# snakers4/mnasnet-pytorch

Measured on AMD Instinct MI355X. Metric: images/sec MNASNet-1.0 224^2 bf16 train step, higher is better.
Workload: dtype bf16; 1 GPU; MNASNet-1.0 (Mnasnet(cut_channels_first=False)+head '512', 1000 classes) fwd+bwd+Adam, bs=256/GPU, 224x224, per-rank BatchNorm; global_batch=256, parallelism=dp1

## Files before the change

### include/mnas.h

```cpp
#ifndef MNAS_H
#define MNAS_H
#include <stdint.h>

#ifdef __cplusplus
extern "C" {
#endif

#define MNAS_OK 0
#define MNAS_EINVAL 10001
#define MNAS_BN_ROWS 8

typedef struct MnasActIn {
    const void*  data;
    const float* scale;
    const float* shift;
} MnasActIn;

typedef struct MnasGradIn {
    const void*  g;
    const void*  y;
    const float* coef;
} MnasGradIn;

int mnas_version(void);
// ... 52 lines not shown

typedef struct MnasConvWgrad {
    int32_t N, Hi, Wi, Ci;
    int32_t Ho, Wo, Co;
    int32_t kh, kw, stride, pad;
    int32_t nsplit;
    MnasActIn  x;
    MnasGradIn dy;
    float* partial;
} MnasConvWgrad;
int mnas_conv_wgrad(const MnasConvWgrad* a, void* stream);
int mnas_conv_wgrad_slabs(int Co, int Ci, int taps);
int mnas_conv_wgrad_instance(const MnasConvWgrad* a, int* out);

int mnas_wgrad_finalize(float* partial, int nsplit, int Co, int Ci, int taps,
                        float* grad, int accumulate, void* stream);

typedef struct MnasPwBwd {
    int32_t M, Ci, Co, nparts;
    MnasActIn  x;
    MnasGradIn dy;
    const void* w;
    const void* resid;
    void*  gin;
    float* wpartial;
    float* red_partial;
    const void*  red_y;
    const float* red_bn;
    const void*  w_fwd;
    const float* b_fwd;
    int32_t gin_masked;
    int32_t seg_px;
} MnasPwBwd;
int mnas_pw_bwd(const MnasPwBwd* a, void* stream);
int mnas_pw_bwd_supported(int Ci, int Co);
int mnas_pw_bwd_tile_pixels(int Ci, int Co);
int mnas_pw_bwd_slices(int Ci, int Co);
int mnas_pw_bwd_forms(int Ci, int Co);
int mnas_pw_bwd_instance(const MnasPwBwd* a, int* out);

typedef struct MnasDwFwd {
    int32_t N, H, W, C, k;
    int32_t nparts;
    MnasActIn in;
    const float* w;
    const float* bias;
    void*  out;
    float* stats;
    int32_t stride, reserved;
} MnasDwFwd;
int mnas_dw_fwd(const MnasDwFwd* a, void* stream);
int mnas_dw_geometry(int N, int H, int W, int C, int k, int which, int* out);
int mnas_dw_rows(int N, int H, int W, int C, int k, int nparts, int which);

typedef struct MnasDwBwd {
    int32_t N, H, W, C, k;
    int32_t nparts;
    MnasActIn  x;
    MnasGradIn dy;
    const float* w;
    void*  gin;
    float* wpartial;
    const float* red_bn;
    float* red_partial;
    int32_t phase;
    int32_t stride;
    int32_t g_masked, reserved;
} MnasDwBwd;
int mnas_dw_bwd(const MnasDwBwd* a, void* stream);
int mnas_dw_wgrad_finalize(float* wpartial, int nparts, int C, int k, float* grad, int accumulate,
                           void* stream);

typedef struct MnasStemFwd {
    int32_t N, H, W, Ho, Wo, Co;
    int32_t nparts;
    const float* x;
    const void*  w;
    const float* bias;
    void*  out;
    float* stats;
    const float* in_affine;
    int32_t in_u8, reserved;
} MnasStemFwd;
int mnas_stem_fwd(const MnasStemFwd* a, void* stream);
typedef struct MnasStemWgrad {
    int32_t N, H, W, Ho, Wo, Co;
    int32_t nparts;
    const float* x;
    MnasGradIn dy;
    float* partial;
    const float* in_affine;
    int32_t in_u8, reserved;
} MnasStemWgrad;
int mnas_stem_wgrad(const MnasStemWgrad* a, void* stream);
int mnas_stem_parts(int which, int N, int H, int W, int Co);
int mnas_stem_dgrad(const MnasGradIn* dy, const float* w, int N, int H, int W, int Ho, int Wo, int Co, const float* in_affine,
                    float* dx, void* stream);

int mnas_bn_fwd_finalize(const float* partial, int nparts, int C, double count,
                         const float* gamma, const float* beta,
                         float* running_mean, float* running_var, int64_t* num_batches_tracked,
                         float momentum, float eps, int training, float* bnbuf, void* stream);
int mnas_bn_bwd_reduce(const void* g, const void* y, const float* bnbuf, int64_t rows, int C,
                       int nparts, float* partial, void* stream);
int mnas_dy_materialize(const MnasGradIn* d, int64_t rows, int C, void* out_bf16, void* stream);
int mnas_bn_bwd_finalize(const float* partial, int nparts, int C, double count,
// ... 411 lines not shown
```

### mnasnet_pytorch_amd/_lib.py

```python
from __future__ import annotations

import ctypes as C
import os

import torch

_HERE = os.path.dirname(os.path.abspath(__file__))
ABI_VERSION = 8
LIB_PATH = os.environ.get("MNAS_LIB_PATH") or os.path.join(_HERE, "csrc", "libmnas_hip.so")

c_void_p, c_int, c_float, c_double, c_int64 = C.c_void_p, C.c_int, C.c_float, C.c_double, C.c_int64


class MnasActIn(C.Structure):
    _fields_ = [("data", c_void_p), ("scale", c_void_p), ("shift", c_void_p)]


class MnasGradIn(C.Structure):
    _fields_ = [("g", c_void_p), ("y", c_void_p), ("coef", c_void_p)]


class MnasConvGemm(C.Structure):
    _fields_ = [("mode", C.c_int32), ("N", C.c_int32), ("Hi", C.c_int32), ("Wi", C.c_int32), ("Ci", C.c_int32),
                ("Ho", C.c_int32), ("Wo", C.c_int32), ("Co", C.c_int32), ("kh", C.c_int32), ("kw", C.c_int32),
# ... 323 lines not shown
                                        c_void_p]),
    "mnas_head_cross_entropy_metrics": (c_int, [c_void_p, c_void_p, c_int, c_int, c_int64, c_void_p, c_void_p, c_void_p, c_void_p,
                                                C.POINTER(c_int), c_int, c_void_p, c_void_p, c_void_p]),
    "mnas_head_metrics": (c_int, [c_void_p, c_void_p, c_int, c_int, C.POINTER(c_int), c_int, c_void_p, c_void_p, c_void_p,
                                  c_void_p]),
    "mnas_head_cross_entropy_soft": (c_int, [c_void_p, c_void_p, c_void_p, c_void_p, c_float, c_int, c_int, c_int64, c_void_p,
                                             c_void_p, c_void_p, c_void_p, C.POINTER(c_int), c_int, c_void_p, c_void_p, c_void_p]),
    "mnas_head_cross_entropy_kd": (c_int, [c_void_p, c_void_p, c_void_p, c_void_p, c_float, c_void_p, c_void_p, c_float, c_float, c_int,
                                           c_int, c_int64, c_void_p, c_void_p, c_void_p, c_void_p, c_void_p, C.POINTER(c_int), c_int,
                                           c_void_p, c_void_p, c_void_p]),
    "mnas_mlabel_scratch_bytes": (c_int64, [c_int]),
    "mnas_mlabel_bce": (c_int, [c_void_p, c_void_p, c_void_p, c_int, c_int, c_int, c_float, c_float, c_void_p, c_void_p, c_void_p,
                                c_void_p, c_int64, c_int64, c_int64, c_void_p]),
    "mnas_mlabel_metrics": (c_int, [c_void_p, c_void_p, c_int, c_int, c_void_p, c_void_p, c_void_p, c_int64, c_int64, c_int64,
                                    c_void_p]),
    "mnas_mlabel_hard_dice": (c_int, [c_void_p, c_void_p, c_int, c_int, c_float, c_int, c_void_p, c_void_p, c_void_p]),
    "mnas_se_scale": (c_int, [C.POINTER(MnasActIn), c_void_p, c_int, c_int, c_int, c_void_p, c_void_p]),
    "mnas_se_bwd_reduce": (c_int, [c_void_p, C.POINTER(MnasActIn), c_void_p, c_int, c_int, c_int, c_void_p, c_void_p, c_void_p]),
    "mnas_se_scratch_bytes": (c_int64, [c_int, c_int, c_int]),
    "mnas_se_bwd_apply": (c_int, [c_void_p, c_void_p, c_void_p, c_int, c_int, c_int, c_void_p, c_void_p, c_void_p, c_void_p, c_void_p]),
    "mnas_se_bwd_apply_cols": (c_int, [c_int, c_int, c_int]),
    "mnas_se_gate": (c_int, [c_void_p, c_int, c_int, c_void_p, c_void_p]),
    "mnas_se_proj_finalize": (c_int, [c_void_p, c_int, c_int, c_int, c_int, c_void_p, c_void_p, c_void_p, c_int, c_void_p, c_void_p]),
    "mnas_stem_dgrad": (c_int, [c_void_p, c_void_p] + [c_int] * 6 + [c_void_p] * 3),
    "mnas_se_fc_supported": (c_int, [c_int, c_int]),
    "mnas_se_fc_fwd": (c_int, [c_void_p] * 5 + [c_int] * 3 + [c_void_p] * 4),
    "mnas_se_fc_bwd": (c_int, [c_void_p] * 5 + [c_int] * 3 + [c_void_p] * 6 + [c_int, c_void_p]),
    "mnas_conv_gemm_gate_ok": (c_int, [c_int, c_int, c_int, c_int]),
    "mnas_graph_create": (c_int, [C.POINTER(MnasOp), c_int, C.POINTER(c_void_p), c_int, C.POINTER(c_void_p), C.POINTER(c_int)]),
    "mnas_graph_launch": (c_int, [c_void_p, c_void_p]),
    "mnas_graph_destroy": (c_int, [c_void_p]),
    "mnas_version": (c_int, []),
    "mnas_arch": (C.c_char_p, []),
    "mnas_workspace_bytes": (c_int64, [c_int, c_int, c_int, c_int]),
    "mnas_conv_gemm": (c_int, [C.POINTER(MnasConvGemm), c_void_p]),
    "mnas_conv_gemm_route": (c_int, [C.POINTER(MnasConvGemm), C.POINTER(c_int)]),
    "mnas_conv_gemm_instance": (c_int, [C.POINTER(MnasConvGemm), C.POINTER(c_int)]),
    "mnas_conv_gemm_tile_pixels": (c_int, [c_int, c_int, c_int]),
    "mnas_conv_gemm_parts": (c_int, [c_int, c_int, c_int, c_int, c_int]),
    "mnas_conv_wgrad": (c_int, [C.POINTER(MnasConvWgrad), c_void_p]),
    "mnas_conv_wgrad_instance": (c_int, [C.POINTER(MnasConvWgrad), C.POINTER(c_int)]),
    "mnas_conv_wgrad_slabs": (c_int, [c_int, c_int, c_int]),
    "mnas_wgrad_finalize": (c_int, [c_void_p, c_int, c_int, c_int, c_int, c_void_p, c_int, c_void_p]),
    "mnas_pw_bwd": (c_int, [C.POINTER(MnasPwBwd), c_void_p]),
    "mnas_pw_bwd_supported": (c_int, [c_int, c_int]),
    "mnas_pw_bwd_forms": (c_int, [c_int, c_int]),
    "mnas_pw_bwd_instance": (c_int, [C.POINTER(MnasPwBwd), C.POINTER(c_int)]),
    "mnas_pw_bwd_tile_pixels": (c_int, [c_int, c_int]),
    "mnas_pw_bwd_slices": (c_int, [c_int, c_int]),
    "mnas_dw_fwd": (c_int, [C.POINTER(MnasDwFwd), c_void_p]),
    "mnas_dw_bwd": (c_int, [C.POINTER(MnasDwBwd), c_void_p]),
    "mnas_dw_rows": (c_int, [c_int, c_int, c_int, c_int, c_int, c_int, c_int]),
    "mnas_dw_geometry": (c_int, [c_int, c_int, c_int, c_int, c_int, c_int, C.POINTER(c_int)]),
    "mnas_dw_wgrad_finalize": (c_int, [c_void_p, c_int, c_int, c_int, c_void_p, c_int, c_void_p]),
    "mnas_stem_fwd": (c_int, [C.POINTER(MnasStemFwd), c_void_p]),
    "mnas_stem_wgrad": (c_int, [C.POINTER(MnasStemWgrad), c_void_p]),
    "mnas_bn_fwd_finalize": (c_int, [c_void_p, c_int, c_int, c_double, c_void_p, c_void_p, c_void_p, c_void_p,
                                     c_void_p, c_float, c_float, c_int, c_void_p, c_void_p]),
    "mnas_bn_bwd_reduce": (c_int, [c_void_p, c_void_p, c_void_p, c_int64, c_int, c_int, c_void_p, c_void_p]),
    "mnas_tconv_dgrad": (c_int, [C.POINTER(MnasTconvDgrad), c_void_p]),
    "mnas_tconv_dgrad_instance": (c_int, [C.POINTER(MnasTconvDgrad), C.POINTER(c_int)]),
    "mnas_tconv_supported": (c_int, [c_int, c_int, c_int, c_int]),
    "mnas_tconv_parts": (c_int, [c_int, c_int, c_int, c_int, c_int]),
    "mnas_bwd_post": (c_int, [C.POINTER(MnasBwdPost), c_void_p]),
    "mnas_bwd_post_frozen": (c_int, [C.POINTER(MnasBwdPostFrozen), c_void_p]),
    "mnas_bn_bwd_finalize_frozen": (c_int, [c_void_p, c_int, c_int, c_void_p, c_void_p, c_void_p, c_void_p, c_int, c_void_p]),
    "mnas_bn_frozen_tables": (c_int, [c_void_p, c_int, c_void_p]),
    "mnas_dy_materialize": (c_int, [C.POINTER(MnasGradIn), c_int64, c_int, c_void_p, c_void_p]),
    "mnas_bn_bwd_finalize": (c_int, [c_void_p, c_int, c_int, c_double, c_void_p, c_void_p, c_void_p, c_int, c_void_p]),
    "mnas_add_act": (c_int, [C.POINTER(MnasActIn), C.POINTER(MnasActIn), c_int64, c_int, c_void_p, c_void_p, c_int,
                             c_void_p]),
    "mnas_pool_act": (c_int, [C.POINTER(MnasActIn), c_int, c_int, c_int, c_void_p, c_void_p]),
    "mnas_pool_bwd": (c_int, [c_void_p, c_int, c_int, c_int, c_void_p, c_void_p]),
    "mnas_nchw_f32_to_nhwc_bf16": (c_int, [c_void_p, c_void_p, c_int, c_int, c_int, c_void_p]),
    "mnas_pack_weights": (c_int, [c_void_p, c_int, c_int, c_int, c_int, c_int, c_void_p, c_void_p]),
    "mnas_pack_weights_batch": (c_int, [c_void_p, c_int, c_void_p]),
    "mnas_packed_bytes": (c_int64, [c_int, c_int, c_int, c_int, c_int]),
    "mnas_adam_step": (c_int, [c_void_p, c_void_p, c_void_p, c_void_p, c_int64, c_float, c_float, c_float, c_float,
                               c_float, c_int, c_float, c_void_p]),
    "mnas_rmsprop_step": (c_int, [c_void_p, c_void_p, c_void_p, c_void_p, c_int64, c_float, c_float, c_float, c_float, c_float,
                                  c_float, c_void_p]),
    "mnas_sgd_step": (c_int, [c_void_p, c_void_p, c_void_p, c_int64, c_float, c_float, c_float, c_float, c_int, c_int, c_float,
                              c_void_p]),
    "mnas_grad_sqnorm": (c_int, [c_void_p, c_int64, c_float, c_void_p, c_int, C.POINTER(c_int), c_void_p]),
    "mnas_adam_step_ex": (c_int, [c_void_p, c_void_p, c_void_p, c_void_p, c_int64, c_float, c_float, c_float, c_float,
                                  c_float, c_int, c_float, C.POINTER(MnasOptExtra), c_void_p]),
    "mnas_rmsprop_step_ex": (c_int, [c_void_p, c_void_p, c_void_p, c_void_p, c_int64, c_float, c_float, c_float, c_float, c_float,
                                     c_float, C.POINTER(MnasOptExtra), c_void_p]),
    "mnas_sgd_step_ex": (c_int, [c_void_p, c_void_p, c_void_p, c_int64, c_float, c_float, c_float, c_float, c_int, c_int, c_float,
                                 C.POINTER(MnasOptExtra), c_void_p]),
    "mnas_adam_step_seg": (c_int, [c_void_p, c_void_p, c_void_p, c_void_p, c_float, c_float, c_float, c_int, c_float,
                                   C.POINTER(MnasOptSegs), C.POINTER(MnasOptExtra), c_void_p]),
    "mnas_rmsprop_step_seg": (c_int, [c_void_p, c_void_p, c_void_p, c_void_p, c_float, c_float, c_float, c_float,
                                      C.POINTER(MnasOptSegs), C.POINTER(MnasOptExtra), c_void_p]),
    "mnas_sgd_step_seg": (c_int, [c_void_p, c_void_p, c_void_p, c_float, c_float, c_int, c_int, c_float,
                                  C.POINTER(MnasOptSegs), C.POINTER(MnasOptExtra), c_void_p]),
    "mnas_run_ops": (c_int, [C.POINTER(MnasOp), c_int, c_void_p, C.POINTER(c_int)]),
    "mnas_run_ops_multi": (c_int, [C.POINTER(MnasOp), c_int, C.POINTER(c_void_p), c_int, C.POINTER(c_int)]),
    "mnas_event_create": (c_int, [C.POINTER(c_void_p)]),
    "mnas_event_destroy": (c_int, [c_void_p]),
    "mnas_event_record": (c_int, [c_void_p, c_void_p]),
    "mnas_event_elapsed_ms": (c_int, [c_void_p, c_void_p, C.POINTER(c_float)]),
    "mnas_probe_copy": (c_int, [c_void_p, c_void_p, c_int64, c_void_p]),
    "mnas_probe_valu": (c_int, [c_void_p, c_int, c_int, c_void_p]),
    "mnas_probe_copy4": (c_int, [c_void_p, c_void_p, c_int64, c_int, c_void_p]),
    "mnas_probe_read": (c_int, [c_void_p, c_void_p, c_int64, c_int, c_void_p]),
# ... 50 lines not shown
```

### mnasnet_pytorch_amd/csrc/mnas_common.h

```cpp
#pragma once
#include <hip/hip_runtime.h>
#include <stdint.h>
#include "../../include/mnas.h"

#define MNAS_WAVE 64
typedef __attribute__((ext_vector_type(8))) short bf16x8_t;
typedef __attribute__((ext_vector_type(4))) float f32x4_t;

#ifdef MNAS_DIAG
#include <cstdlib>
static inline int mnas_diag_env(const char* name, int dflt) { const char* e = getenv(name); return e ? atoi(e) : dflt; }
#else
#define mnas_diag_env(name, dflt) (dflt)
#endif
#define MNAS_SWITCH(fn, expr) int fn() { static int on = -1; if (on < 0) on = (expr); return on; }

#define MNAS_CHECK_LAUNCH() do { hipError_t e_ = hipGetLastError(); if (e_ != hipSuccess) return (int)e_; } while (0)

#ifndef MNAS_EARLY
#define MNAS_EARLY 1
#endif
template <class F>
__device__ __forceinline__ void mnas_fill_table(float* dst, int n, int tid, int nth, F f) {
#if MNAS_EARLY
// ... 121 lines not shown
    if (rcp == 0.f) return n / d;
    int q = (int)((float)n * rcp);
    const int r = n - q * d;
    q += (r >= d) ? 1 : 0;
    q -= (r < 0) ? 1 : 0;
    return q;
}

typedef __attribute__((ext_vector_type(4))) short mnas_s4_t;
typedef __attribute__((address_space(3))) mnas_s4_t* mnas_lds_s4_ptr;
__device__ __forceinline__ bf16x8_t mnas_tr_frag(const uint16_t* tile, int ld, int row0, int col0, int lane) {
    const int i = lane & 15, g = lane >> 4;
    const uint16_t* p = tile + (row0 + g * 8 + (i >> 2)) * ld + col0 + (i & 3) * 4;
    const mnas_s4_t lo = __builtin_amdgcn_ds_read_tr16_b64_v4i16((mnas_lds_s4_ptr)p);
    const mnas_s4_t hi = __builtin_amdgcn_ds_read_tr16_b64_v4i16((mnas_lds_s4_ptr)(p + 4 * ld));
    return __builtin_shufflevector(lo, hi, 0, 1, 2, 3, 4, 5, 6, 7);
}

typedef unsigned int u32x2_t __attribute__((ext_vector_type(2)));
typedef unsigned int u32x4_t __attribute__((ext_vector_type(4)));
__device__ __forceinline__ void st_u1(void* p, uint32_t v, bool nt) {
    if (nt) __builtin_nontemporal_store(v, (uint32_t*)p); else *(uint32_t*)p = v;
}
__device__ __forceinline__ void st_u2(void* p, uint2 v, bool nt) {
    if (nt) __builtin_nontemporal_store((u32x2_t){v.x, v.y}, (u32x2_t*)p); else *(uint2*)p = v;
}
__device__ __forceinline__ void st_u4(void* p, uint4 v, bool nt) {
    if (nt) __builtin_nontemporal_store((u32x4_t){v.x, v.y, v.z, v.w}, (u32x4_t*)p); else *(uint4*)p = v;
}
#define MNAS_NT_IGEMM_FWD 1
#define MNAS_NT_IGEMM_DGRAD 2
#define MNAS_NT_DW_FWD 4
#define MNAS_NT_DW_BWD 8
#define MNAS_NT_PW_BWD 16
#define MNAS_NT_ADD_ACT 32
#define MNAS_NT_STEM 64
#define MNAS_NT_PWF 128
int mnas_nt_mask();
int mnas_pwf_enabled();
int mnas_pwf_parts(int M, int Ci, int Co);
int mnas_pwf_forward(const MnasConvGemm* c, void* stream, int* inst = nullptr);
int mnas_stem_fwd_band(const MnasStemFwd* c, void* stream);
int mnas_stem_wgrad_band(const MnasStemWgrad* c, void* stream);
int mnas_dimg_parts(int mode, int N, int Hi, int Wi, int Ci, int Ho, int Wo, int Co, int kh, int kw, int stride, int pad);
int mnas_dimg_run(const MnasConvGemm* c, void* stream, int* inst = nullptr);
int mnas_c3r_parts(int mode, int N, int Hi, int Wi, int Ci, int Ho, int Wo, int Co, int kh, int kw, int stride, int pad);
int mnas_c3r_run(const MnasConvGemm* c, void* stream, int* inst = nullptr);
int mnas_pwd_enabled();
int mnas_pwd_parts(int M, int Ci, int Co);
int mnas_pwd_dgrad(const MnasConvGemm* c, void* stream, int* inst = nullptr);
int mnas_dw2_rows(int N, int H, int W, int C, int k, int nparts, int which);
int mnas_dw2_fwd(const MnasDwFwd* c, void* stream);
int mnas_dw2_bwd(const MnasDwBwd* c, void* stream);
int mnas_pws_enabled();
int mnas_pws_parts(int mode, int M, int K, int N);
int mnas_pws_run(const MnasConvGemm* c, void* stream, int* inst = nullptr);
int mnas_pws_accepts(const MnasConvGemm* c);
int mnas_pws_gate_ok(int M, int K, int N);
int mnas_c3x_ok(int N, int Hi, int Wi, int Ci, int Ho, int Wo, int Co, int kh, int kw, int stride, int pad);
int mnas_c3x_run(const MnasConvGemm* c, void* stream, int* inst = nullptr);
int mnas_tcx_ok(int Ho, int Wo, int Co, int Ci);
int mnas_tcx_parts(int N, int Ho, int Wo, int Co, int Ci);
int mnas_tcx_dgrad(const MnasTconvDgrad* c, void* stream, int* inst = nullptr);
int mnas_tcr_ok(int Ho, int Wo, int Co, int Ci);
int mnas_tcr_parts(int N, int Ho, int Wo, int Co, int Ci);
int mnas_tcr_dgrad(const MnasTconvDgrad* c, void* stream, int* inst = nullptr);
int mnas_pwx_parts(int M, int Ci, int Co);
int mnas_pwx_forward(const MnasConvGemm* c, void* stream, int* inst = nullptr);

__device__ __forceinline__ float wave_sum(float v) {
#pragma unroll
    for (int o = 32; o > 0; o >>= 1) v += __shfl_xor(v, o, 64);
    return v;
}

template <int NT>
__device__ __forceinline__ void mnas_stats_store(const float (&s1)[NT][4], const float (&s2)[NT][4], float* red, int c0, int Co,
                                                 float* stats, int tid, int wave, int l15, int lg) {
    constexpr int NB = NT * 16;
#pragma unroll
    for (int t = 0; t < NT; ++t)
#pragma unroll
        for (int r = 0; r < 4; ++r) {
            float x1 = s1[t][r], x2 = s2[t][r];
#pragma unroll
            for (int o = 1; o < 16; o <<= 1) { x1 += __shfl_xor(x1, o, 64); x2 += __shfl_xor(x2, o, 64); }
            if (l15 == 0) {
                red[(wave * 2 + 0) * NB + t * 16 + lg * 4 + r] = x1;
                red[(wave * 2 + 1) * NB + t * 16 + lg * 4 + r] = x2;
            }
        }
    __syncthreads();
    for (int i = tid; i < 2 * NB; i += 256) {
        const int r = i / NB, cl = i % NB, c = c0 + cl;
        const float v = ((red[(0 * 2 + r) * NB + cl] + red[(1 * 2 + r) * NB + cl]) + red[(2 * 2 + r) * NB + cl]) + red[(3 * 2 + r) * NB + cl];
        if (c < Co) stats[((size_t)r * Co + c) * gridDim.x + blockIdx.x] = v;
    }
}
__device__ __forceinline__ void mnas_colsum_store(const float* r1, const float* r2, float* fin, int nc, int tcols, int step, int c0,
                                                  int nvalid, int C, float* out, int tid) {
    __syncthreads();
#pragma unroll
    for (int j = 0; j < 8; ++j) { fin[tid * 16 + j] = r1[j]; fin[tid * 16 + 8 + j] = r2[j]; }
    __syncthreads();
    for (int i = tid; i < 2 * nc; i += 256) {
        const int r = i / nc, c = i % nc;
// ... 13 lines not shown
```

### mnasnet_pytorch_amd/csrc/mnas_dw.hip

```cpp
#include "mnas_common.h"
#ifndef MNAS_DW_XFILL
#define MNAS_DW_XFILL 1
#endif

#ifndef MNAS_DW_NODMA
#define MNAS_DW_NODMA 0
#endif
#ifndef MNAS_DW_NOCOMP
#define MNAS_DW_NOCOMP 0
#endif
#ifndef MNAS_DW_NOBARRIER
#define MNAS_DW_NOBARRIER 0
#endif
__device__ __forceinline__ void dw_step_barrier() {
    if (MNAS_DW_NOBARRIER) asm volatile("s_waitcnt vmcnt(0)" ::: "memory");
    else dma_barrier();
}

#ifndef MNAS_DW_XCD
#define MNAS_DW_XCD 1
#endif
#ifndef MNAS_DW_RA
#define MNAS_DW_RA 1
#endif
// ... 561 lines not shown
    a->nthreads = ((sx * cpw + 63) / 64) * 64;
    a->iw = iw;
    a->strips_x = (W + sx * DW_BW - 1) / (sx * DW_BW);
    a->cblocks = (cps + cpw - 1) / cpw;
    a->items = N * a->strips_x * a->cblocks;
    a->rc = iw * cgn;
    a->nb = (a->rc + 63) / 64;
    if (a->nb > 2 * (a->nthreads / 64)) return false;
    *g = gg;
    return true;
}
static bool dw_choose(int N, int H, int W, int C, int k, int form, DwArgs* a, int* g) {
    DwArgs a4, a2;
    const int nrings = dw_rings(form);
    if (mnas_diag_env("MNAS_DW_CPW", 0) > 0 && dw_force(N, H, W, C, k, nrings, a, g)) return true;
    const bool ok4 = dw_pick(N, H, W, C, k, nrings, 8, &a4), ok2 = dw_pick(N, H, W, C, k, nrings, 4, &a2);
    if (!ok4 && !ok2) return false;
    if (ok2 && (!ok4 || 0.93f * a2.score > a4.score)) { *a = a2; *g = 2; }
    else { *a = a4; *g = 4; }
    return true;
}
static bool dw_finish(DwArgs* a, int nparts) {
    if (nparts < a->cblocks) return false;
    int g = nparts < a->items ? nparts : a->items;
    a->geff = g / a->cblocks * a->cblocks;
    return a->geff >= a->cblocks;
}
static const int dw_form_of[4] = {-1, 0, 1, 2};
extern "C" int mnas_dw_rows(int N, int H, int W, int C, int k, int nparts, int which) {
    if (which == 4 || which == 7) return mnas_dw2_rows(N, H, W, C, k, nparts, which - 4);
    if (which < 0 || which > 3) return -1;
    DwArgs a;
    int g;
    if (!dw_choose(N, H, W, C, k, dw_form_of[which], &a, &g) || !dw_finish(&a, nparts)) return -1;
    return a.geff / a.cblocks;
}

extern "C" int mnas_dw_geometry(int N, int H, int W, int C, int k, int which, int* out) {
    if (which < 0 || which > 3 || !out) return MNAS_EINVAL;
    DwArgs a;
    int g;
    if (!dw_choose(N, H, W, C, k, dw_form_of[which], &a, &g)) return MNAS_EINVAL;
    out[0] = a.cpw; out[1] = a.sx; out[2] = a.nthreads; out[3] = a.strips_x; out[4] = a.cblocks;
    out[5] = dw_rings(dw_form_of[which]) * 2 * g * a.rc * 16; out[6] = g;
    return MNAS_OK;
}

extern "C" int mnas_dw_fwd(const MnasDwFwd* c, void* stream) {
    if (!c || (c->k != 3 && c->k != 5) || (c->C & 7) || c->nparts < 1 || c->stride < 0 || c->stride > 2) return MNAS_EINVAL;
    if (c->stride == 2) return mnas_dw2_fwd(c, stream);
    DwArgs a;
    int g;
    if (!dw_choose(c->N, c->H, c->W, c->C, c->k, -1, &a, &g) || !dw_finish(&a, c->nparts)) return MNAS_EINVAL;
    a.nt = (mnas_nt_mask() & MNAS_NT_DW_FWD) ? 1 : 0;
    size_t lds = (size_t)2 * g * a.rc * 16;
    const size_t red_need = (size_t)a.sx * 2 * 2 * a.cpw * sizeof(float);
    if (lds < red_need) lds = red_need;
    hipStream_t s = (hipStream_t)stream;
#define MNAS_DWF(K_, G_) do { if (c->in.scale) hipLaunchKernelGGL((k_dw_fwd<K_, G_, true>), dim3(a.geff), dim3(a.nthreads), lds, s, a, c->in, c->w, c->bias, \
                                            (uint32_t*)c->out, c->stats); \
                              else hipLaunchKernelGGL((k_dw_fwd<K_, G_, false>), dim3(a.geff), dim3(a.nthreads), lds, s, a, c->in, c->w, c->bias, \
                                            (uint32_t*)c->out, c->stats); } while (0)
    if (c->k == 3) { if (g == 4) MNAS_DWF(3, 4); else MNAS_DWF(3, 2); }
    else { if (g == 4) MNAS_DWF(5, 4); else MNAS_DWF(5, 2); }
#undef MNAS_DWF
    MNAS_CHECK_LAUNCH();
    return MNAS_OK;
}

template <int KS, bool DG, bool WG, bool RED, int G, bool GM>
static void dw_bwd_launch(const DwArgs& a, size_t lds, hipStream_t s, const MnasDwBwd* c) {
    if constexpr (WG) {
        if (!c->x.scale) {
            hipLaunchKernelGGL((k_dw_bwd<KS, DG, WG, RED, G, GM, false>), dim3(a.geff), dim3(a.nthreads), lds, s, a, c->x, c->dy, c->w,
                               (uint32_t*)c->gin, c->wpartial, c->red_partial, c->red_bn);
            return;
        }
    }
    hipLaunchKernelGGL((k_dw_bwd<KS, DG, WG, RED, G, GM, true>), dim3(a.geff), dim3(a.nthreads), lds, s, a, c->x, c->dy, c->w,
                       (uint32_t*)c->gin, c->wpartial, c->red_partial, c->red_bn);
}

extern "C" int mnas_dw_bwd(const MnasDwBwd* c, void* stream) {
    if (!c || (c->k != 3 && c->k != 5) || (c->C & 7) || c->nparts < 1 || c->phase < 0 || c->phase > 2) return MNAS_EINVAL;
    if (c->stride < 0 || c->stride > 2) return MNAS_EINVAL;
    if (c->stride == 2) return mnas_dw2_bwd(c, stream);
    hipStream_t s = (hipStream_t)stream;
    if (!c->x.data || !c->dy.g) return MNAS_EINVAL;
    const bool red = c->red_bn != nullptr && c->red_partial != nullptr;
    const bool want_dg = c->phase != 2, want_wg = c->phase != 1;
    const int nrings = dw_rings(c->phase);
    DwArgs a;
    int g;
    if (!dw_choose(c->N, c->H, c->W, c->C, c->k, c->phase, &a, &g) || !dw_finish(&a, c->nparts)) return MNAS_EINVAL;
    a.nt = (mnas_nt_mask() & MNAS_NT_DW_BWD) ? 1 : 0;
    size_t lds = (size_t)nrings * 2 * g * a.rc * 16;
    const size_t red_need = (size_t)a.sx * (want_wg ? c->k * c->k : 2) * 2 * a.cpw * sizeof(float);
    if (lds < red_need) lds = red_need;
#define MNAS_DWB(K_, DG_, WG_, R_, G_) dw_bwd_launch<K_, DG_, WG_, R_, G_, false>(a, lds, s, c)
#define MNAS_DWB_G(K_, DG_, WG_, R_) do { if (g == 4) MNAS_DWB(K_, DG_, WG_, R_, 4); else MNAS_DWB(K_, DG_, WG_, R_, 2); } while (0)
    if (c->g_masked) {
        if (!(want_dg && want_wg && red)) return MNAS_EINVAL;
        if (c->k == 3) { if (g == 4) dw_bwd_launch<3, true, true, true, 4, true>(a, lds, s, c); else dw_bwd_launch<3, true, true, true, 2, true>(a, lds, s, c); }
        else { if (g == 4) dw_bwd_launch<5, true, true, true, 4, true>(a, lds, s, c); else dw_bwd_launch<5, true, true, true, 2, true>(a, lds, s, c); }
        MNAS_CHECK_LAUNCH();
        return MNAS_OK;
    }
    if (c->k == 3) {
        if (want_dg && want_wg) { if (red) MNAS_DWB_G(3, true, true, true); else MNAS_DWB_G(3, true, true, false); }
        else if (want_dg) { if (red) MNAS_DWB_G(3, true, false, true); else MNAS_DWB_G(3, true, false, false); }
        else MNAS_DWB_G(3, false, true, false);
    } else {
        if (want_dg && want_wg) { if (red) MNAS_DWB_G(5, true, true, true); else MNAS_DWB_G(5, true, true, false); }
        else if (want_dg) { if (red) MNAS_DWB_G(5, true, false, true); else MNAS_DWB_G(5, true, false, false); }
        else MNAS_DWB_G(5, false, true, false);
    }
#undef MNAS_DWB_G
#undef MNAS_DWB
    MNAS_CHECK_LAUNCH();
    return MNAS_OK;
}
```

Measured before the change: 25910 images/sec.

## Add whole-plane LDS depthwise kernels for 7x7 and 14x14 stride-1 layers

Adds forward and backward depthwise conv kernels that stage an entire 7x7 or 14x14 image plane per channel group in LDS via async global-to-LDS loads. Each block loops persistently over images, prefetching the next image while it computes the current one. The backward kernel fuses input-grad, weight-grad and BN reduction partials. The existing strip-based path is bypassed when the shape qualifies, aiming to cut halo reloads and launch inefficiency on small spatial layers. In exchange it uses large LDS footprints that limit occupancy, and it adds new code paths that could differ numerically, for example in the order of reductions.

```diff
diff --git a/include/mnas.h b/include/mnas.h
--- a/include/mnas.h
+++ b/include/mnas.h
@@ -128,6 +128,8 @@
 int mnas_dw_fwd(const MnasDwFwd* a, void* stream);
 int mnas_dw_geometry(int N, int H, int W, int C, int k, int which, int* out);
 int mnas_dw_rows(int N, int H, int W, int C, int k, int nparts, int which);
+int mnas_dw_plane(int on);
+int mnas_dw_plane_takes(int N, int H, int W, int C, int k, int which);
 
 typedef struct MnasDwBwd {
     int32_t N, H, W, C, k;
diff --git a/mnasnet_pytorch_amd/_lib.py b/mnasnet_pytorch_amd/_lib.py
--- a/mnasnet_pytorch_amd/_lib.py
+++ b/mnasnet_pytorch_amd/_lib.py
@@ -399,6 +399,8 @@
     "mnas_dw_bwd": (c_int, [C.POINTER(MnasDwBwd), c_void_p]),
     "mnas_dw_rows": (c_int, [c_int, c_int, c_int, c_int, c_int, c_int, c_int]),
     "mnas_dw_geometry": (c_int, [c_int, c_int, c_int, c_int, c_int, c_int, C.POINTER(c_int)]),
+    "mnas_dw_plane": (c_int, [c_int]),
+    "mnas_dw_plane_takes": (c_int, [c_int, c_int, c_int, c_int, c_int, c_int]),
     "mnas_dw_wgrad_finalize": (c_int, [c_void_p, c_int, c_int, c_int, c_void_p, c_int, c_void_p]),
     "mnas_stem_fwd": (c_int, [C.POINTER(MnasStemFwd), c_void_p]),
     "mnas_stem_wgrad": (c_int, [C.POINTER(MnasStemWgrad), c_void_p]),
diff --git a/mnasnet_pytorch_amd/csrc/mnas_common.h b/mnasnet_pytorch_amd/csrc/mnas_common.h
--- a/mnasnet_pytorch_amd/csrc/mnas_common.h
+++ b/mnasnet_pytorch_amd/csrc/mnas_common.h
@@ -197,6 +197,10 @@
 int mnas_dw2_rows(int N, int H, int W, int C, int k, int nparts, int which);
 int mnas_dw2_fwd(const MnasDwFwd* c, void* stream);
 int mnas_dw2_bwd(const MnasDwBwd* c, void* stream);
+int mnas_dwp_fwd_ok(int H, int W, int k);
+int mnas_dwp_fwd(const MnasDwFwd* c, int rows, void* stream);
+int mnas_dwp_bwd_ok(int H, int W, int k);
+int mnas_dwp_bwd(const MnasDwBwd* c, int rows, void* stream);
 int mnas_pws_enabled();
 int mnas_pws_parts(int mode, int M, int K, int N);
 int mnas_pws_run(const MnasConvGemm* c, void* stream, int* inst = nullptr);
diff --git a/mnasnet_pytorch_amd/csrc/mnas_dw.hip b/mnasnet_pytorch_amd/csrc/mnas_dw.hip
--- a/mnasnet_pytorch_amd/csrc/mnas_dw.hip
+++ b/mnasnet_pytorch_amd/csrc/mnas_dw.hip
@@ -637,6 +637,7 @@
     DwArgs a;
     int g;
     if (!dw_choose(c->N, c->H, c->W, c->C, c->k, -1, &a, &g) || !dw_finish(&a, c->nparts)) return MNAS_EINVAL;
+    if (c->stats && a.strips_x == 1 && mnas_dwp_fwd_ok(c->H, c->W, c->k)) return mnas_dwp_fwd(c, a.geff / a.cblocks, stream);
     a.nt = (mnas_nt_mask() & MNAS_NT_DW_FWD) ? 1 : 0;
     size_t lds = (size_t)2 * g * a.rc * 16;
     const size_t red_need = (size_t)a.sx * 2 * 2 * a.cpw * sizeof(float);
@@ -682,6 +683,8 @@
     size_t lds = (size_t)nrings * 2 * g * a.rc * 16;
     const size_t red_need = (size_t)a.sx * (want_wg ? c->k * c->k : 2) * 2 * a.cpw * sizeof(float);
     if (lds < red_need) lds = red_need;
+    if (want_dg && want_wg && red && a.strips_x == 1 && c->dy.y && c->dy.coef && c->gin && c->wpartial && mnas_dwp_bwd_ok(c->H, c->W, c->k))
+        return mnas_dwp_bwd(c, a.geff / a.cblocks, stream);
 #define MNAS_DWB(K_, DG_, WG_, R_, G_) dw_bwd_launch<K_, DG_, WG_, R_, G_, false>(a, lds, s, c)
 #define MNAS_DWB_G(K_, DG_, WG_, R_) do { if (g == 4) MNAS_DWB(K_, DG_, WG_, R_, 4); else MNAS_DWB(K_, DG_, WG_, R_, 2); } while (0)
     if (c->g_masked) {
diff --git a/mnasnet_pytorch_amd/csrc/mnas_dwp.hip b/mnasnet_pytorch_amd/csrc/mnas_dwp.hip
--- /dev/null
+++ b/mnasnet_pytorch_amd/csrc/mnas_dwp.hip
@@ -0,0 +1,481 @@
+#include "mnas_common.h"
+
+typedef float f2 __attribute__((ext_vector_type(2)));
+__device__ __forceinline__ f2 p_f2fma(f2 a, f2 b, f2 c) { return __builtin_elementwise_fma(a, b, c); }
+__device__ __forceinline__ f2 p_f2bf(uint32_t u) { f2 r; r.x = bf_lo(u); r.y = bf_hi(u); return r; }
+
+#define DWP_THREADS 256
+
+template <int KS, int HW>
+struct DwpGeo {
+    static constexpr int PAD = KS / 2;
+    static constexpr int CPW = HW == 14 ? 16 : 32;
+    static constexpr int CG = CPW / 4;
+    static constexpr int S = (HW + PAD) | 1;
+    static constexpr int PLANE_PX = PAD + HW * S;
+    static constexpr int NCH = HW * HW * CG;
+    static constexpr int NB = (NCH + 63) / 64;
+    static constexpr int NJ = (NB + DWP_THREADS / 64 - 1) / (DWP_THREADS / 64);
+    static constexpr int NE = HW * HW * CPW;
+    static constexpr size_t SB = (size_t)HW * 4 * CPW * sizeof(float);
+    static constexpr size_t LDS = (size_t)PLANE_PX * CPW * 8 + (size_t)NE * 4 + SB;
+    static_assert(S - HW >= PAD && DWP_THREADS % CPW == 0 && HW * CPW <= DWP_THREADS, "plane geometry");
+};
+
+struct DwpArgs {
+    int N, C, rows, pcb;
+    int slots;
+    int nt;
+};
+
+template <int KS, int HW, bool HC>
+__global__ __launch_bounds__(DWP_THREADS, 3) void k_dwp_fwd(DwpArgs a, MnasActIn in, const float* __restrict__ w,
+                                                            const float* __restrict__ bias, uint32_t* __restrict__ out,
+                                                            float* __restrict__ stats) {
+    typedef DwpGeo<KS, HW> G;
+    constexpr int PAD = G::PAD, CPW = G::CPW, S = G::S, WIN = HW + KS - 1, CB = 2 * CPW;
+    extern __shared__ __attribute__((aligned(16))) unsigned char smem[];
+    f2* plane = (f2*)smem;
+    uint32_t* raw = (uint32_t*)(plane + G::PLANE_PX * CPW);
+    float* sb = (float*)(raw + G::NE);
+    const int tid = threadIdx.x, lane = tid & 63;
+    const int wave = __builtin_amdgcn_readfirstlane(tid >> 6);
+    const int bid = (int)xcd_remap(blockIdx.x, gridDim.x);
+    const int slot = bid / a.pcb, c0 = (bid - slot * a.pcb) * CB;
+    const int cp = tid % CPW, row = tid / CPW;
+    const bool active = row < HW;
+    const int ch = c0 + 2 * cp;
+    const bool ch_ok = ch < a.C;
+    const int C8 = a.C >> 3;
+    const unsigned voff = ((unsigned)(active ? row : 0) * HW * a.C + (ch_ok ? ch : 0)) * 2;
+
+    int goff[G::NJ];
+    bool ok[G::NJ];
+#pragma unroll
+    for (int j = 0; j < G::NJ; ++j) {
+        const int q = (j * (DWP_THREADS / 64) + wave) * 64 + lane;
+        const int px = q / G::CG, cgl = q - px * G::CG;
+        ok[j] = q < G::NCH && (c0 + cgl * 8) < a.C;
+        goff[j] = px * C8 + cgl;
+    }
+    auto dma = [&](int n) {
+        const uint4* src = (const uint4*)in.data + (size_t)n * HW * HW * C8 + (c0 >> 3);
+#pragma unroll
+        for (int j = 0; j < G::NJ; ++j) {
+            const int b = j * (DWP_THREADS / 64) + wave;
+            if (b >= G::NB) continue;
+            if (ok[j]) __builtin_amdgcn_global_load_lds((mnas_gbl_ptr)(src + goff[j]), (mnas_lds_ptr)(raw + b * 256), 16, 0, 0);
+        }
+    };
+    int col = slot, n = slot;
+    dma(n);
+
+    const f2 zero2 = {0.f, 0.f};
+    f2 wt[KS * KS], b2, cs = {1.f, 1.f}, ct = zero2;
+#pragma unroll
+    for (int t = 0; t < KS * KS; ++t) {
+        wt[t].x = ch_ok ? w[(size_t)t * a.C + ch] : 0.f;
+        wt[t].y = ch_ok ? w[(size_t)t * a.C + ch + 1] : 0.f;
+    }
+    b2.x = (bias && ch_ok) ? bias[ch] : 0.f;
+    b2.y = (bias && ch_ok) ? bias[ch + 1] : 0.f;
+    if (HC && ch_ok) { cs.x = in.scale[ch]; cs.y = in.scale[ch + 1]; ct.x = in.shift[ch]; ct.y = in.shift[ch + 1]; }
+
+    for (int e = tid; e < (PAD + HW * (S - HW)) * CPW; e += DWP_THREADS) {
+        const int h = e / CPW, c = e - h * CPW;
+        int p = h;
+        if (h >= PAD) { const int y = (h - PAD) / (S - HW), j = (h - PAD) - y * (S - HW); p = PAD + y * S + HW + j; }
+        plane[p * CPW + c] = zero2;
+    }
+    auto fold = [&](int pcol) {
+        for (int i = tid; i < 2 * CB; i += DWP_THREADS) {
+            const int r = i / CB, cl = i - r * CB, c = c0 + cl;
+            float v = sb[r * CB + cl];
+            for (int y = 1; y < HW; ++y) v += sb[(y * 2 + r) * CB + cl];
+            if (c < a.C) stats[((size_t)r * a.C + c) * a.rows + pcol] = v;
+        }
+    };
+
+    f2 s1 = zero2, s2 = zero2;
+    int pend = -1;
+    bool have = true;
+    while (have) {
+        int ncol = col, nn = n + a.rows;
+        if (nn >= a.N) { ncol = col + a.slots; nn = ncol; }
+        const bool nhave = ncol < a.rows;
+        const bool last = ncol != col;
+        dma_barrier();
+        if (pend >= 0) { fold(pend); pend = -1; }
+        if (active) {
+            uint32_t rv[HW];
+#pragma unroll
+            for (int y = 0; y < HW; ++y) rv[y] = raw[(y * HW + row) * CPW + cp];
+#pragma unroll
+            for (int y = 0; y < HW; ++y) {
+                f2 v = p_f2bf(rv[y]);
+                if (HC) {
+                    v = p_f2fma(v, cs, ct);
+                    v.x = fmaxf(v.x, 0.f); v.y = fmaxf(v.y, 0.f);
+                }
+                plane[(PAD + y * S + row) * CPW + cp] = v;
+            }
+        }
+        __syncthreads();
+        if (nhave) dma(nn);
+        if (active) {
+            f2 acc[HW];
+#pragma unroll
+            for (int ox = 0; ox < HW; ++ox) acc[ox] = b2;
+#pragma unroll
+            for (int ky = 0; ky < KS; ++ky) {
+                const int iy = row + ky - PAD;
+                if (iy >= 0 && iy < HW) {
+                    const f2* rp = plane + (size_t)(iy * S) * CPW + cp;
+                    f2 xr[WIN];
+#pragma unroll
+                    for (int x = 0; x < WIN; ++x) xr[x] = rp[x * CPW];
+#pragma unroll
+                    for (int ox = 0; ox < HW; ++ox)
+#pragma unroll
+                        for (int kx = 0; kx < KS; ++kx) acc[ox] = p_f2fma(wt[ky * KS + kx], xr[ox + kx], acc[ox]);
+                }
+            }
+            if (ch_ok) {
+                uint32_t* ob = out + (size_t)n * HW * HW * a.C / 2;
+#pragma unroll
+                for (int ox = 0; ox < HW; ++ox) {
+                    const f2 v = acc[ox];
+                    s1 += v;
+                    s2 = p_f2fma(v, v, s2);
+                    st_u1((char*)(ob + (size_t)ox * (a.C / 2)) + voff, pack_bf16(v.x, v.y), a.nt);
+                }
+            }
+            if (last) {
+                sb[(row * 2 + 0) * CB + 2 * cp] = s1.x; sb[(row * 2 + 0) * CB + 2 * cp + 1] = s1.y;
+                sb[(row * 2 + 1) * CB + 2 * cp] = s2.x; sb[(row * 2 + 1) * CB + 2 * cp + 1] = s2.y;
+                s1 = zero2; s2 = zero2;
+            }
+        }
+        if (last) pend = col;
+        col = ncol; n = nn; have = nhave;
+    }
+    __syncthreads();
+    if (pend >= 0) fold(pend);
+}
+
+#ifndef DWP_NH514
+#define DWP_NH514 2
+#endif
+#ifndef DWP_BWD_WAVES
+#define DWP_BWD_WAVES 2
+#endif
+template <int KS, int HW>
+struct DwpBwdGeo {
+    typedef DwpGeo<KS, HW> F;
+    static constexpr int NV = KS * KS + 2;
+    static constexpr size_t PLANE = (size_t)F::PLANE_PX * F::CPW * 8, RAW = (size_t)F::NE * 4;
+    static constexpr size_t PARK = (size_t)(DWP_THREADS / 64) * NV * 2 * F::CPW * sizeof(float);
+    static constexpr int NH = (KS == 5 && HW == 14) ? DWP_NH514 : 1;
+    static constexpr bool WT_LDS = KS == 5;
+    static constexpr size_t WT = WT_LDS ? (size_t)KS * KS * F::CPW * 8 : 0;
+    static constexpr size_t LDS = PLANE + 2 * RAW + PARK + WT;
+};
+
+template <int KS, int HW, bool HC, bool GM>
+__global__ __launch_bounds__(DWP_THREADS, DWP_BWD_WAVES) void k_dwp_bwd(DwpArgs a, MnasActIn x, MnasGradIn d, const float* __restrict__ w,
+                                                            uint32_t* __restrict__ gin, float* __restrict__ wpartial,
+                                                            float* __restrict__ red_partial, const float* __restrict__ red_bn) {
+    typedef DwpGeo<KS, HW> G;
+    typedef DwpBwdGeo<KS, HW> B;
+    constexpr int PAD = G::PAD, CPW = G::CPW, S = G::S, WIN = HW + KS - 1, CB = 2 * CPW, KK = KS * KS, NV = B::NV;
+    extern __shared__ __attribute__((aligned(16))) unsigned char smem[];
+    f2* plane = (f2*)smem;
+    uint32_t* rawg = (uint32_t*)(plane + G::PLANE_PX * CPW);
+    uint32_t* rawy = rawg + G::NE;
+    float* park = (float*)(rawy + G::NE);
+    f2* wlds = (f2*)(park + (DWP_THREADS / 64) * NV * CB);
+    const int tid = threadIdx.x, lane = tid & 63;
+    const int wave = __builtin_amdgcn_readfirstlane(tid >> 6);
+    const int bid = (int)xcd_remap(blockIdx.x, gridDim.x);
+    const int slot = bid / a.pcb, c0 = (bid - slot * a.pcb) * CB;
+    const int cp = tid % CPW, row = tid / CPW;
+    const bool active = row < HW;
+    const int ch = c0 + 2 * cp;
+    const bool ch_ok = ch < a.C;
+    const int C8 = a.C >> 3;
+    const uint32_t* xg = (const uint32_t*)x.data;
+    const unsigned voff = ((unsigned)(active ? row : 0) * HW * a.C + (ch_ok ? ch : 0)) * 2;
+
+    int goff[G::NJ];
+    bool ok[G::NJ];
+#pragma unroll
+    for (int j = 0; j < G::NJ; ++j) {
+        const int q = (j * (DWP_THREADS / 64) + wave) * 64 + lane;
+        const int px = q / G::CG, cgl = q - px * G::CG;
+        ok[j] = q < G::NCH && (c0 + cgl * 8) < a.C;
+        goff[j] = px * C8 + cgl;
+    }
+    auto dma = [&](int n) {
+        const size_t base = (size_t)n * HW * HW * C8 + (c0 >> 3);
+        const uint4 *sg = (const uint4*)d.g + base, *sy = (const uint4*)d.y + base;
+#pragma unroll
+        for (int j = 0; j < G::NJ; ++j) {
+            const int b = j * (DWP_THREADS / 64) + wave;
+            if (b >= G::NB) continue;
+            if (ok[j]) {
+                __builtin_amdgcn_global_load_lds((mnas_gbl_ptr)(sg + goff[j]), (mnas_lds_ptr)(smem + B::PLANE + (size_t)b * 1024), 16, 0, 0);
+                __builtin_amdgcn_global_load_lds((mnas_gbl_ptr)(sy + goff[j]), (mnas_lds_ptr)(smem + B::PLANE + B::RAW + (size_t)b * 1024), 16, 0, 0);
+            }
+        }
+    };
+    auto xrow = [&](int n) { return xg + (size_t)n * HW * HW * a.C / 2; };
+    int col = slot, n = slot;
+    uint32_t xraw[HW];
+    dma(n);
+    {
+        const uint32_t* p = xrow(n);
+#pragma unroll
+        for (int ox = 0; ox < HW; ++ox) xraw[ox] = *(const uint32_t*)((const char*)(p + (size_t)ox * (a.C / 2)) + voff);
+    }
+
+    const f2 zero2 = {0.f, 0.f};
+    f2 wt[B::WT_LDS ? 1 : KK], wacc[KK], cf[3], ms = zero2, mt = zero2, cs = {1.f, 1.f}, ct = zero2, ris = zero2, rmu = zero2;
+#pragma unroll
+    for (int t = 0; t < KK; ++t) wacc[t] = zero2;
+    if constexpr (B::WT_LDS) {
+        for (int e = tid; e < KK * CPW; e += DWP_THREADS) {
+            const int t = e / CPW, c = c0 + 2 * (e - t * CPW);
+            f2 v = zero2;
+            if (c < a.C) { v.x = w[(size_t)(KK - 1 - t) * a.C + c]; v.y = w[(size_t)(KK - 1 - t) * a.C + c + 1]; }
+            wlds[e] = v;
+        }
+    } else {
+#pragma unroll
+        for (int t = 0; t < KK; ++t) {
+            wt[t].x = ch_ok ? w[(size_t)(KK - 1 - t) * a.C + ch] : 0.f;
+            wt[t].y = ch_ok ? w[(size_t)(KK - 1 - t) * a.C + ch + 1] : 0.f;
+        }
+    }
+#pragma unroll
+    for (int r = 0; r < 3; ++r) {
+        cf[r].x = ch_ok ? d.coef[(size_t)(r + 2) * a.C + ch] : 0.f;
+        cf[r].y = ch_ok ? d.coef[(size_t)(r + 2) * a.C + ch + 1] : 0.f;
+    }
+    if (!GM && ch_ok) { ms.x = d.coef[ch]; ms.y = d.coef[ch + 1]; mt.x = d.coef[(size_t)a.C + ch]; mt.y = d.coef[(size_t)a.C + ch + 1]; }
+    if (x.scale != nullptr && ch_ok) { cs.x = x.scale[ch]; cs.y = x.scale[ch + 1]; ct.x = x.shift[ch]; ct.y = x.shift[ch + 1]; }
+    if (ch_ok) {
+        ris.x = red_bn[6 * a.C + ch]; ris.y = red_bn[6 * a.C + ch + 1];
+        rmu.x = -red_bn[5 * a.C + ch] * ris.x; rmu.y = -red_bn[5 * a.C + ch + 1] * ris.y;
+    }
+    for (int e = tid; e < (PAD + HW * (S - HW)) * CPW; e += DWP_THREADS) {
+        const int h = e / CPW, c = e - h * CPW;
+        int p = h;
+        if (h >= PAD) { const int y = (h - PAD) / (S - HW), j = (h - PAD) - y * (S - HW); p = PAD + y * S + HW + j; }
+        plane[p * CPW + c] = zero2;
+    }
+    auto fold = [&](int pcol) {
+        for (int i = tid; i < NV * CB; i += DWP_THREADS) {
+            const int v = i / CB, cl = i - v * CB, c = c0 + cl;
+            float acc = park[i];
+#pragma unroll
+            for (int wv = 1; wv < DWP_THREADS / 64; ++wv) acc += park[wv * NV * CB + i];
+            if (c < a.C) {
+                if (v < 2) red_partial[((size_t)v * a.C + c) * a.rows + pcol] = acc;
+                else wpartial[((size_t)pcol * KK + (v - 2)) * a.C + c] = acc;
+            }
+        }
+    };
+
+    f2 s1 = zero2, s2 = zero2;
+    int pend = -1;
+    bool have = true;
+    while (have) {
+        int ncol = col, nn = n + a.rows;
+        if (nn >= a.N) { ncol = col + a.slots; nn = ncol; }
+        const bool nhave = ncol < a.rows;
+        const bool last = ncol != col;
+        dma_barrier();
+        if (pend >= 0) { fold(pend); pend = -1; }
+        if (active) {
+            uint32_t gr[HW], yr[HW];
+#pragma unroll
+            for (int y = 0; y < HW; ++y) { gr[y] = rawg[(y * HW + row) * CPW + cp]; yr[y] = rawy[(y * HW + row) * CPW + cp]; }
+#pragma unroll
+            for (int y = 0; y < HW; ++y) {
+                const f2 gv = p_f2bf(gr[y]), yv = p_f2bf(yr[y]);
+                f2 dz = gv;
+                if constexpr (!GM) {
+                    const f2 z = p_f2fma(yv, ms, mt);
+                    dz.x = (z.x > 0.f) ? gv.x : 0.f;
+                    dz.y = (z.y > 0.f) ? gv.y : 0.f;
+                }
+                plane[(PAD + y * S + row) * CPW + cp] = p_f2fma(cf[0], dz, p_f2fma(cf[1], yv, cf[2]));
+            }
+        }
+        __syncthreads();
+        if (nhave) dma(nn);
+        if (active) {
+            f2 xa[WIN];
+#pragma unroll
+            for (int i = 0; i < WIN; ++i) xa[i] = zero2;
+#pragma unroll
+            for (int ox = 0; ox < HW; ++ox) {
+                f2 v = p_f2bf(xraw[ox]);
+                if (HC) {
+                    v = p_f2fma(v, cs, ct);
+                    v.x = fmaxf(v.x, 0.f); v.y = fmaxf(v.y, 0.f);
+                }
+                xa[ox + PAD] = v;
+            }
+            uint32_t* gp = gin + (size_t)n * HW * HW * a.C / 2;
+#pragma unroll
+            for (int h = 0; h < B::NH; ++h) {
+                constexpr int OW = HW / B::NH;
+                f2 A[OW];
+#pragma unroll
+                for (int ox = 0; ox < OW; ++ox) A[ox] = zero2;
+#pragma unroll
+                for (int dd = 0; dd < KS; ++dd) {
+                    const int iy = row + dd - PAD;
+                    if (iy >= 0 && iy < HW) {
+                        const f2* rp = plane + (size_t)(iy * S + h * OW) * CPW + cp;
+                        f2 dr[OW + KS - 1], wr[KS];
+#pragma unroll
+                        for (int i = 0; i < OW + KS - 1; ++i) dr[i] = rp[i * CPW];
+#pragma unroll
+                        for (int kx = 0; kx < KS; ++kx) {
+                            if constexpr (B::WT_LDS) wr[kx] = wlds[(dd * KS + kx) * CPW + cp];
+                            else wr[kx] = wt[dd * KS + kx];
+                        }
+#pragma unroll
+                        for (int ox = 0; ox < OW; ++ox)
+#pragma unroll
+                            for (int kx = 0; kx < KS; ++kx) A[ox] = p_f2fma(wr[kx], dr[ox + kx], A[ox]);
+#pragma unroll
+                        for (int ox = 0; ox < OW; ++ox)
+#pragma unroll
+                            for (int kx = 0; kx < KS; ++kx)
+                                wacc[(KS - 1 - dd) * KS + kx] = p_f2fma(dr[ox + PAD], xa[h * OW + ox + kx], wacc[(KS - 1 - dd) * KS + kx]);
+                    }
+                }
+                if (ch_ok) {
+#pragma unroll
+                    for (int ox = 0; ox < OW; ++ox) {
+                        const int gx = h * OW + ox;
+                        const uint32_t pk = pack_bf16(A[ox].x, A[ox].y);
+                        st_u1((char*)(gp + (size_t)gx * (a.C / 2)) + voff, pk, a.nt);
+                        const f2 gq = p_f2bf(pk), yq = p_f2bf(xraw[gx]), z = xa[gx + PAD];
+                        f2 dz;
+                        dz.x = (z.x > 0.f) ? gq.x : 0.f;
+                        dz.y = (z.y > 0.f) ? gq.y : 0.f;
+                        s1 += dz;
+                        s2 = p_f2fma(dz, p_f2fma(yq, ris, rmu), s2);
+                    }
+                }
+            }
+        }
+        if (nhave) {
+            const uint32_t* p = xrow(nn);
+#pragma unroll
+            for (int ox = 0; ox < HW; ++ox) xraw[ox] = *(const uint32_t*)((const char*)(p + (size_t)ox * (a.C / 2)) + voff);
+        }
+        if (last) {
+            f2 sv[NV];
+            sv[0] = s1; sv[1] = s2;
+#pragma unroll
+            for (int t = 0; t < KK; ++t) sv[t + 2] = wacc[t];
+#pragma unroll
+            for (int v = 0; v < NV; ++v) {
+#pragma unroll
+                for (int o = CPW; o < 64; o <<= 1) {
+                    sv[v].x += __shfl_xor(sv[v].x, o, 64);
+                    sv[v].y += __shfl_xor(sv[v].y, o, 64);
+                }
+            }
+            if (lane < CPW) {
+                float* p = park + (size_t)wave * NV * CB + 2 * cp;
+#pragma unroll
+                for (int v = 0; v < NV; ++v) { p[v * CB] = sv[v].x; p[v * CB + 1] = sv[v].y; }
+            }
+            s1 = zero2; s2 = zero2;
+#pragma unroll
+            for (int t = 0; t < KK; ++t) wacc[t] = zero2;
+            pend = col;
+        }
+        col = ncol; n = nn; have = nhave;
+    }
+    __syncthreads();
+    if (pend >= 0) fold(pend);
+}
+
+#ifndef DWP_FWD_RESIDENT
+#define DWP_FWD_RESIDENT 768
+#endif
+#ifndef DWP_BWD_RESIDENT
+#define DWP_BWD_RESIDENT 512
+#endif
+static int g_dw_plane = 1;
+extern "C" int mnas_dw_plane(int on) {
+    const int prev = g_dw_plane;
+    g_dw_plane = on ? 1 : 0;
+    return prev;
+}
+static bool dwp_shape(int H, int W, int k) { return H == W && (H == 7 || H == 14) && (k == 3 || k == 5); }
+int mnas_dwp_fwd_ok(int H, int W, int k) { return g_dw_plane && dwp_shape(H, W, k); }
+int mnas_dwp_bwd_ok(int H, int W, int k) { return g_dw_plane && dwp_shape(H, W, k); }
+extern "C" int mnas_dw_plane_takes(int N, int H, int W, int C, int k, int which) {
+    if (which < 0 || which > 1 || N < 1 || C < 8 || (C & 7)) return 0;
+    if (!(which == 0 ? mnas_dwp_fwd_ok(H, W, k) : mnas_dwp_bwd_ok(H, W, k))) return 0;
+    int geo[7];
+    if (mnas_dw_geometry(N, H, W, C, k, which, geo) != MNAS_OK) return 0;
+    return geo[3] == 1;
+}
+static void dwp_args(DwpArgs* a, int N, int H, int C, int rows, int resident) {
+    const int cb = H == 14 ? 32 : 64;
+    a->N = N; a->C = C; a->rows = rows;
+    a->pcb = (C + cb - 1) / cb;
+    const int fit = resident / a->pcb;
+    a->slots = rows < fit ? rows : (fit < 1 ? 1 : fit);
+}
+
+template <int KS, int HW>
+static void dwp_launch(const MnasDwFwd* c, const DwpArgs& a, hipStream_t s) {
+    typedef DwpGeo<KS, HW> G;
+    const dim3 grid(a.slots * a.pcb), block(DWP_THREADS);
+    if (c->in.scale) hipLaunchKernelGGL((k_dwp_fwd<KS, HW, true>), grid, block, G::LDS, s, a, c->in, c->w, c->bias, (uint32_t*)c->out, c->stats);
+    else hipLaunchKernelGGL((k_dwp_fwd<KS, HW, false>), grid, block, G::LDS, s, a, c->in, c->w, c->bias, (uint32_t*)c->out, c->stats);
+}
+int mnas_dwp_fwd(const MnasDwFwd* c, int rows, void* stream) {
+    if (!c->stats || rows < 1 || rows > c->N || !mnas_dwp_fwd_ok(c->H, c->W, c->k)) return MNAS_EINVAL;
+    DwpArgs a;
+    dwp_args(&a, c->N, c->H, c->C, rows, DWP_FWD_RESIDENT);
+    a.nt = (mnas_nt_mask() & MNAS_NT_DW_FWD) ? 1 : 0;
+    hipStream_t s = (hipStream_t)stream;
+    if (c->H == 14) { if (c->k == 3) dwp_launch<3, 14>(c, a, s); else dwp_launch<5, 14>(c, a, s); }
+    else { if (c->k == 3) dwp_launch<3, 7>(c, a, s); else dwp_launch<5, 7>(c, a, s); }
+    MNAS_CHECK_LAUNCH();
+    return MNAS_OK;
+}
+
+template <int KS, int HW>
+static void dwp_launch_bwd(const MnasDwBwd* c, const DwpArgs& a, hipStream_t s) {
+    typedef DwpBwdGeo<KS, HW> G;
+    const dim3 grid(a.slots * a.pcb), block(DWP_THREADS);
+#define DWP_BWD_GO(HC_, GM_) hipLaunchKernelGGL((k_dwp_bwd<KS, HW, HC_, GM_>), grid, block, G::LDS, s, a, c->x, c->dy, c->w, (uint32_t*)c->gin, \
+                                              c->wpartial, c->red_partial, c->red_bn)
+    if (c->x.scale) { if (c->g_masked) DWP_BWD_GO(true, true); else DWP_BWD_GO(true, false); }
+    else { if (c->g_masked) DWP_BWD_GO(false, true); else DWP_BWD_GO(false, false); }
+#undef DWP_BWD_GO
+}
+int mnas_dwp_bwd(const MnasDwBwd* c, int rows, void* stream) {
+    if (c->phase != 0 || !c->red_bn || !c->red_partial || !c->wpartial || !c->gin || !c->dy.y || !c->dy.coef) return MNAS_EINVAL;
+    if (rows < 1 || rows > c->N || !mnas_dwp_bwd_ok(c->H, c->W, c->k)) return MNAS_EINVAL;
+    DwpArgs a;
+    dwp_args(&a, c->N, c->H, c->C, rows, DWP_BWD_RESIDENT);
+    a.nt = (mnas_nt_mask() & MNAS_NT_DW_BWD) ? 1 : 0;
+    hipStream_t s = (hipStream_t)stream;
+    if (c->H == 14) { if (c->k == 3) dwp_launch_bwd<3, 14>(c, a, s); else dwp_launch_bwd<5, 14>(c, a, s); }
+    else { if (c->k == 3) dwp_launch_bwd<3, 7>(c, a, s); else dwp_launch_bwd<5, 7>(c, a, s); }
+    MNAS_CHECK_LAUNCH();
+    return MNAS_OK;
+}
```

After: 26170 images/sec (median of 6 runs). No clear change (+1.0%).
